# nomic-ai/contrastors

Measured on AMD Instinct MI355X. Metric: query-doc pairs/sec (whole node), nomic-bert-2048 seq128 global-batch 16384, higher is better.
Workload: dtype bf16

## Files before the change

contrastors_amd/csrc/gemm_bf16_v6.hip:

```cpp
#include "cx_common.h"
#include "../../include/contrastors_hip.h"
#include "gemm_params.h"
#include <type_traits>

namespace {

#ifndef CX_V6_HI_EARLY
#define CX_V6_HI_EARLY 1
#endif
#ifndef CX_V6_OPAQUE
#define CX_V6_OPAQUE 1
#endif
#ifndef CX_V6_NT
#define CX_V6_NT 3
#endif
template <int J>
__device__ __forceinline__ void v6_dma_m0(uint32_t slot_base) {
    asm volatile("s_add_u32 m0, %0, %1" ::"s"(slot_base), "n"(J * 4096) : "memory", "scc");
}
__device__ __forceinline__ void v6_dma_ld(uint32_t off, const bf16_t* base) {
    asm volatile("global_load_lds_dwordx4 %0, %1" ::"v"(off), "s"(base) : "memory");
}
template <int J>
__device__ __forceinline__ void v6_dma_full(uint32_t slot_base, uint32_t off, const bf16_t* base) {
    asm volatile("s_add_u32 m0, %0, %1\n\ts_nop 0\n\tglobal_load_lds_dwordx4 %2, %3" ::"s"(slot_base), "n"(J * 4096), "v"(off),
                 "s"(base) : "memory", "scc");
}
typedef unsigned int cx_u32x4 __attribute__((ext_vector_type(4)));
__device__ __forceinline__ void gst_nt(void* ptr, uint4 v) {
    cx_u32x4 t = {v.x, v.y, v.z, v.w};
    __builtin_nontemporal_store(t, reinterpret_cast<cx_u32x4*>(ptr));
}
__device__ __forceinline__ uint4 gld_nt(const void* ptr) {
    const cx_u32x4 t = __builtin_nontemporal_load(reinterpret_cast<const cx_u32x4*>(ptr));
    return make_uint4(t.x, t.y, t.z, t.w);
}
#if CX_V6_NT & 1
#define gst(ptr, v) gst_nt((ptr), (v))
#else
#define gst(ptr, v) (*reinterpret_cast<uint4*>(ptr) = (v))
#endif
#if CX_V6_NT & 2
#define gld(ptr) gld_nt(ptr)
#else
#define gld(ptr) (*reinterpret_cast<const uint4*>(ptr))
#endif

typedef __attribute__((address_space(3))) void* lds_void_ptr;
typedef const __attribute__((address_space(1))) void* glb_void_ptr;

constexpr int BM6 = 256, BN6 = 256, BK6 = 64;
constexpr int XS6 = 32768;
constexpr int LDS6 = 5 * XS6;

struct Frags6 {
    bf16x8_t w[8], x[8];
};

#include "gemm_v6_acc.inc"

template <int I0, int I1, class F>
CX_DEVICE void v6_static_for(F&& f) {
    if constexpr (I0 < I1) {
        f(std::integral_constant<int, I0>{});
        v6_static_for<I0 + 1, I1>(f);
    }
}

template <int EPI, int DBG = 0>
__global__ __launch_bounds__(256, 1) __attribute__((amdgpu_waves_per_eu(1, 1))) void gemm_bf16_v6_kernel(GemmParams p) {
    extern __shared__ __attribute__((aligned(16))) char dsm[];
    constexpr bool IS_SWIGLU_BWD = EPI == GEMM_EPI_SWIGLU_BWD || EPI == GEMM_EPI_SWIGLU_BWD_AG;
    constexpr bool AG = EPI == GEMM_EPI_SWIGLU_BWD_AG;
    constexpr bool SAVEG = EPI == GEMM_EPI_SWIGLU_G;
    long long t_begin = 0, n_ktiles = 0;
    if constexpr (DBG != 0) t_begin = (long long)__builtin_amdgcn_s_memtime();
    long long ph[9] = {0, 0, 0, 0, 0, 0, 0, 0, 0}, t_last = t_begin, kt0_cyc = 0;
#define CX_PH(i_)                                                              \
    do {                                                                       \
        if constexpr ((DBG & 128) != 0) {                                      \
            const long long now_ = (long long)__builtin_amdgcn_s_memtime();    \
            ph[(i_)] += now_ - t_last;                                         \
            t_last = now_;                                                     \
        }                                                                      \
    } while (0)
    const int tid = threadIdx.x;
    const int lane = tid & 63;
    const int wave = __builtin_amdgcn_readfirstlane(tid >> 6);
    const int l15 = lane & 15, g4 = lane >> 4;
    const int wm = wave >> 1, wn = wave & 1;
    const int nk = p.K / BK6;
    const int per_xcd = gridDim.x >> 3;
    const int xcd = blockIdx.x & 7, idx = blockIdx.x >> 3;
    const int gn = p.sup_n > 0 ? p.sup_n : 1, gm = 8 / gn;
    const int xi = xcd / gn, xj = xcd - xi * gn;
    const int m_lo = p.tiles_m * xi / gm, m_hi = p.tiles_m * (xi + 1) / gm;
    const int n_lo = p.tiles_n * xj / gn, n_wd = p.tiles_n * (xj + 1) / gn - n_lo;
    const int nloc = (m_hi - m_lo) * n_wd;
    auto tile_of = [&](int round) {
        const int l = round * per_xcd + idx;
        if (l >= nloc) return -1;
        const int q = l / n_wd;
        return ((m_lo + q) << 8) | (n_lo + (l - q * n_wd));
    };

    uint32_t xoff[8], woff[8];
    const bf16_t* xbase = p.X;
    const bf16_t* wbase = p.W;
    int lx_round = 0, lx_kt = 0, lx_slot = 0;
    int lw_round = 0, lw_kt = 0, lw_slot = 0;
    bool lx_live, lw_live;
    const int first_tile = tile_of(0);
    bool x_clamped = true, w_clamped = true;
    auto x_setup = [&](int tile) {
        const int tm = tile >> 8;
        xbase = p.X + (size_t)tm * BM6 * p.ldx;
        const int rows = p.M - tm * BM6;
        if (rows < BM6 || x_clamped) {
            x_clamped = rows < BM6;
#pragma unroll
            for (int j = 0; j < 8; ++j) {
                const int r = (j * 4 + wave) * 8 + (lane >> 3);
                const int c = (lane & 7) ^ ((r >> 1) & 7);
                const int rr = r < rows ? r : rows - 1;
                xoff[j] = (uint32_t)rr * (uint32_t)p.ldx * 2u + c * 16;
            }
        }
    };
    auto w_setup = [&](int tile) {
        const int tn = tile & 255;
        wbase = p.W + (size_t)tn * BN6 * p.ldw;
        const int rows = p.N - tn * BN6;
        if (rows < BN6 || w_clamped) {
            w_clamped = rows < BN6;
#pragma unroll
            for (int j = 0; j < 8; ++j) {
                const int r = (j * 4 + wave) * 8 + (lane >> 3);
                const int c = (lane & 7) ^ ((r >> 1) & 7);
                const int rr = r < rows ? r : rows - 1;
                woff[j] = (uint32_t)rr * (uint32_t)p.ldw * 2u + c * 16;
            }
        }
    };
    const uint32_t lds0 = (uint32_t)(uintptr_t)(lds_void_ptr)dsm;
    const uint32_t lds_wave = lds0 + wave * 1024;
    uint32_t x_m0 = lds_wave, w_m0 = lds_wave + 3 * XS6;
    auto issue_x_tile = [&]() {
        if constexpr ((DBG & 1) != 0) return;
        v6_dma_full<0>(x_m0, xoff[0], xbase); v6_dma_full<1>(x_m0, xoff[1], xbase); v6_dma_full<2>(x_m0, xoff[2], xbase);
        v6_dma_full<3>(x_m0, xoff[3], xbase); v6_dma_full<4>(x_m0, xoff[4], xbase); v6_dma_full<5>(x_m0, xoff[5], xbase);
        v6_dma_full<6>(x_m0, xoff[6], xbase); v6_dma_full<7>(x_m0, xoff[7], xbase);
    };
    auto issue_w_tile = [&]() {
        if constexpr ((DBG & 1) != 0) return;
        v6_dma_full<0>(w_m0, woff[0], wbase); v6_dma_full<1>(w_m0, woff[1], wbase); v6_dma_full<2>(w_m0, woff[2], wbase);
        v6_dma_full<3>(w_m0, woff[3], wbase); v6_dma_full<4>(w_m0, woff[4], wbase); v6_dma_full<5>(w_m0, woff[5], wbase);
        v6_dma_full<6>(w_m0, woff[6], wbase); v6_dma_full<7>(w_m0, woff[7], wbase);
    };
    auto x_advance = [&]() {
        xbase += BK6;
        lx_slot = lx_slot == 2 ? 0 : lx_slot + 1;
        x_m0 = lds_wave + lx_slot * XS6;
        if (++lx_kt == nk) {
            lx_kt = 0;
            const int t = tile_of(++lx_round);
            lx_live = t >= 0;
            x_setup(lx_live ? t : first_tile);
        }
    };
    auto w_advance = [&]() {
        wbase += BK6;
        lw_slot ^= 1;
        w_m0 = lds_wave + (3 + lw_slot) * XS6;
        if (++lw_kt == nk) {
            lw_kt = 0;
            const int t = tile_of(++lw_round);
            lw_live = t >= 0;
            w_setup(lw_live ? t : first_tile);
        }
    };


    int cp_round = 0;
    int cp_tile = first_tile;
    lx_live = lw_live = cp_tile >= 0;
    if (cp_tile < 0) return;
    x_setup(cp_tile);
    w_setup(cp_tile);
    issue_x_tile();
    x_advance();
    issue_w_tile();
    w_advance();
    issue_x_tile();
    x_advance();
    int xs_slot = 0, ws_slot = 0;

    Frags6 F0, F1;
    auto read_one = [&](Frags6& f, const char* xs, const char* ws, int kk, int i) {
        if constexpr ((DBG & 4) != 0) return;
        if (i < 8)
            f.w[i] = lds_read_frag(ws, tile64_off(wn * 128 + i * 16 + l15, kk * 4 + g4));
        else
            f.x[i - 8] = lds_read_frag(xs, tile64_off(wm * 128 + (i - 8) * 16 + l15, kk * 4 + g4));
    };
    auto mma1 = [&](const Frags6& f, int i) {
        if constexpr ((DBG & 8) != 0) return;
        v6_mfma(i, f.w[i & 7], f.x[i >> 3]);
    };
    auto mma1z = [&](const Frags6& f, int i) {
        if constexpr ((DBG & 8) != 0) return;
        v6_mfma_z(i, f.w[i & 7], f.x[i >> 3]);
    };

#ifndef CX_V6_DMA_SPREAD
#define CX_V6_DMA_SPREAD 4
#endif
#ifndef CX_V6_RD_SPREAD
#define CX_V6_RD_SPREAD 2
#endif
#define CX_SEG(MMA, f, i0, i1, nxt, rxs, rws, rkk, R0, RSP, kind, D0, DSP, J0, ND)                     \
    do {                                                                                              \
        v6_static_for<(i0), (i1)>([&](auto ic_) __attribute__((always_inline)) {                      \
            constexpr int I_ = decltype(ic_)::value;                                                  \
            constexpr bool RD_ = (RSP) > 0 && I_ >= (R0) && (I_ - (R0)) % ((RSP) > 0 ? (RSP) : 1) == 0 && (I_ - (R0)) / ((RSP) > 0 ? (RSP) : 1) < 16; \
            constexpr bool DM_ = (ND) > 0 && I_ >= (D0) && (I_ - (D0)) % (DSP) == 0 && (I_ - (D0)) / (DSP) < (ND); \
            constexpr int J_ = DM_ ? (J0) + (I_ - (D0)) / (DSP) : 0;                                  \
            if constexpr (RD_) read_one(nxt, rxs, rws, rkk, (I_ - (R0)) / ((RSP) > 0 ? (RSP) : 1));   \
            if constexpr (DM_) CX_DMA_M0(kind, J_);                                                   \
            MMA(f, I_);                                                                               \
            if constexpr (DM_) CX_DMA_LD(kind, J_);                                                   \
            __builtin_amdgcn_sched_barrier(0);                                                        \
        });                                                                                           \
    } while (0)
#define CX_DMA_M0(kind, J)                                                       \
    do {                                                                         \
        if constexpr ((kind) == 1 && (DBG & 1) == 0) v6_dma_m0<(J)>(w_m0);        \
        if constexpr ((kind) == 2 && (DBG & 1) == 0) v6_dma_m0<(J)>(x_m0);        \
    } while (0)
#define CX_DMA_LD(kind, J)                                                       \
    do {                                                                         \
        if constexpr ((kind) == 1 && (DBG & 1) == 0) v6_dma_ld(woff[(J)], wbase); \
        if constexpr ((kind) == 2 && (DBG & 1) == 0) v6_dma_ld(xoff[(J)], xbase); \
    } while (0)

    {
        asm volatile("s_waitcnt vmcnt(8)" ::: "memory");
        __builtin_amdgcn_s_barrier();
#pragma unroll
        for (int i = 0; i < 16; ++i) read_one(F0, dsm, dsm + 3 * XS6, 0, i);
    }

    int cp_kt = 0;
    int pxs_slot = 0, pws_slot = 0;
    auto kt_body = [&](auto first) {
        if constexpr (DBG != 0) ++n_ktiles;
        constexpr int RS_ = CX_V6_RD_SPREAD, DS_ = CX_V6_DMA_SPREAD;
        const char* xs = dsm + xs_slot * XS6;
        const char* ws = dsm + (3 + ws_slot) * XS6;
        const int nxs_slot = xs_slot == 2 ? 0 : xs_slot + 1, nws_slot = ws_slot ^ 1;
        if constexpr (decltype(first)::value) {
            CX_SEG(mma1z, F0, 0, 64, F1, xs, ws, 1, RS_ == 2 ? 0 : 1, RS_, 1, RS_ == 2 ? 1 : 17, DS_, 0, 8);
        } else {
            CX_SEG(mma1, F0, 0, 64, F1, xs, ws, 1, RS_ == 2 ? 0 : 1, RS_, 1, RS_ == 2 ? 1 : 17, DS_, 0, 8);
        }
        w_advance();
        CX_SEG(mma1, F1, 0, 32, F0, xs, ws, 0, 0, 0, 2, 0, RS_ == 2 ? 8 : DS_, 0, 4);
        asm volatile("s_waitcnt lgkmcnt(0)" ::: "memory");
        if constexpr ((DBG & 128) != 0) {
            const long long w0_ = (long long)__builtin_amdgcn_s_memtime();
            asm volatile("s_waitcnt vmcnt(4)" ::: "memory");
            const long long w1_ = (long long)__builtin_amdgcn_s_memtime();
            ph[decltype(first)::value ? 0 : 1] += w1_ - w0_;
        } else if constexpr ((DBG & 32) == 0) {
            asm volatile("s_waitcnt vmcnt(4)" ::: "memory");
        }
        if constexpr ((DBG & 2) == 0) __builtin_amdgcn_s_barrier();
        const char* nxs = dsm + nxs_slot * XS6;
        const char* nws = dsm + (3 + nws_slot) * XS6;
        CX_SEG(mma1, F1, 32, 64, F0, nxs, nws, 0, RS_ == 2 ? 32 : 33, RS_, 2, RS_ == 2 ? 33 : 49, RS_ == 2 ? 8 : DS_, 4, 4);
        x_advance();
        if constexpr ((DBG & 128) != 0 && decltype(first)::value) {
            const long long now_ = (long long)__builtin_amdgcn_s_memtime();
            kt0_cyc += now_ - t_last;
        }
        ++cp_kt;
        pxs_slot = xs_slot;
        pws_slot = ws_slot;
        xs_slot = nxs_slot;
        ws_slot = nws_slot;
    };

#pragma unroll 1
    while (cp_tile >= 0) {
        cp_kt = 0;
        kt_body(std::true_type{});
#pragma unroll 1
        while (cp_kt < nk) kt_body(std::false_type{});

        {
            CX_PH(2);
            asm volatile("s_nop 7\n\ts_nop 7\n\ts_nop 7" ::: "memory");
            const int tn = cp_tile & 255, tm = cp_tile >> 8;
            const int m0 = tm * BM6 + wm * 128, n0 = tn * BN6 + wn * 128;
            char* my = ((wave < 2) ? dsm + pxs_slot * XS6 : dsm + (3 + pws_slot) * XS6) + (wave & 1) * 16384;
            constexpr int ROWB = 272;
            auto prow = [&](int q) { return (q >> 1) * 16 + l15; };
            auto pcol = [&](int q) { return (q & 1) * 16 + 4 * g4; };
            auto qoff = [](int q, int rowb) { return (q >> 1) * 16 * rowb + (q & 1) * 32; };
            if constexpr ((DBG & 16) != 0) {
            } else if constexpr (EPI == GEMM_EPI_NONE || EPI == GEMM_EPI_ACT_BWD || EPI == GEMM_EPI_QACT_BWD) {
                constexpr bool ACTB = EPI == GEMM_EPI_ACT_BWD || EPI == GEMM_EPI_QACT_BWD;
                float cs0 = 0.f, cs1 = 0.f, cs2 = 0.f, cs3 = 0.f, cs4 = 0.f, cs5 = 0.f, cs6 = 0.f, cs7 = 0.f;
                constexpr int act_kind = EPI == GEMM_EPI_QACT_BWD ? CX_ACT_QUICK_GELU : CX_ACT_GELU;
                auto mul_grad = [&](uint4& v, const uint4& r) {
#define CX_MG(w_, ca, cb)                                                                              \
    {                                                                                                 \
        const float o0 = bf16lo_to_f32(v.w_) * act_grad(bf16lo_to_f32(r.w_), act_kind);               \
        const float o1 = bf16hi_to_f32(v.w_) * act_grad(bf16hi_to_f32(r.w_), act_kind);               \
        v.w_ = pack_bf16x2(o0, o1);                                                                   \
        ca += bf16lo_to_f32(v.w_);                                                                    \
        cb += bf16hi_to_f32(v.w_);                                                                    \
    }
                    CX_MG(x, cs0, cs1) CX_MG(y, cs2, cs3) CX_MG(z, cs4, cs5) CX_MG(w, cs6, cs7)
#undef CX_MG
                };
                auto flush_colsum = [&]() {
                    if constexpr (ACTB) {
                        float c[8] = {cs0, cs1, cs2, cs3, cs4, cs5, cs6, cs7};
#pragma unroll
                        for (int e = 0; e < 8; ++e) {
                            c[e] += __shfl_xor(c[e], 16, 64);
                            c[e] += __shfl_xor(c[e], 32, 64);
                        }
                        const int n = n0 + (lane & 15) * 8;
                        if (p.colsum_part && lane < 16 && m0 < p.M && n + 8 <= p.N) {
                            float* dst = p.colsum_part + (size_t)(m0 >> 7) * p.N + n;
                            *reinterpret_cast<float4*>(dst) = make_float4(c[0], c[1], c[2], c[3]);
                            *reinterpret_cast<float4*>(dst + 4) = make_float4(c[4], c[5], c[6], c[7]);
                        }
                    }
                };
                const bool add_bias = p.bias != nullptr;
                const bf16_t* resid = reinterpret_cast<const bf16_t*>(p.Out2);
                auto fast_tile = [&](auto with_resid) {
                    constexpr bool RES = decltype(with_resid)::value;
                    const int rrow = lane >> 4, rch = lane & 15;
                    bf16_t* outp = reinterpret_cast<bf16_t*>(p.Out) + (size_t)(m0 + rrow) * p.ldo + n0 + rch * 8;
                    const bf16_t* resp = RES ? resid + (size_t)(m0 + rrow) * p.ldo2 + n0 + rch * 8 : nullptr;
                    const char* rd = my + rrow * ROWB + rch * 16;
                    char* wr = my + prow(0) * ROWB + pcol(0) * 2;
                    uint2 pk[16];
                    auto pack_pass = [&](int b) {
#pragma unroll
                        for (int a = 0; a < 4; ++a) {
                            float blk[16];
                            v6_read_block(4 * b + a, blk);
#pragma unroll
                            for (int q = 0; q < 4; ++q) {
                                pk[a * 4 + q].x = pack_bf16x2(blk[4 * q], blk[4 * q + 1]);
                                pk[a * 4 + q].y = pack_bf16x2(blk[4 * q + 2], blk[4 * q + 3]);
                            }
                        }
                    };
                    auto stage = [&]() {
#pragma unroll
                        for (int a = 0; a < 4; ++a)
#pragma unroll
                            for (int q = 0; q < 4; ++q) *reinterpret_cast<uint2*>(wr + a * 64 + qoff(q, ROWB)) = pk[a * 4 + q];
                    };
                    uint4 r0 = {}, r1 = {}, r2 = {}, r3 = {}, r4 = {}, r5 = {}, r6 = {}, r7 = {};
#define CX_RES_ROWS(b_)                                                                                   \
    r0 = gld(resp + (size_t)((b_) * 32 + 0) * p.ldo2);                          \
    r1 = gld(resp + (size_t)((b_) * 32 + 4) * p.ldo2);                          \
    r2 = gld(resp + (size_t)((b_) * 32 + 8) * p.ldo2);                          \
    r3 = gld(resp + (size_t)((b_) * 32 + 12) * p.ldo2);                         \
    r4 = gld(resp + (size_t)((b_) * 32 + 16) * p.ldo2);                         \
    r5 = gld(resp + (size_t)((b_) * 32 + 20) * p.ldo2);                         \
    r6 = gld(resp + (size_t)((b_) * 32 + 24) * p.ldo2);                         \
    r7 = gld(resp + (size_t)((b_) * 32 + 28) * p.ldo2);
                    auto add_res = [&](uint4& v, const uint4& r) {
                        v.x = pack_bf16x2(bf16lo_to_f32(v.x) + bf16lo_to_f32(r.x), bf16hi_to_f32(v.x) + bf16hi_to_f32(r.x));
                        v.y = pack_bf16x2(bf16lo_to_f32(v.y) + bf16lo_to_f32(r.y), bf16hi_to_f32(v.y) + bf16hi_to_f32(r.y));
                        v.z = pack_bf16x2(bf16lo_to_f32(v.z) + bf16lo_to_f32(r.z), bf16hi_to_f32(v.z) + bf16hi_to_f32(r.z));
                        v.w = pack_bf16x2(bf16lo_to_f32(v.w) + bf16lo_to_f32(r.w), bf16hi_to_f32(v.w) + bf16hi_to_f32(r.w));
                    };
                    auto one_pass = [&](auto bc) {
                        constexpr int b = decltype(bc)::value;
                        uint4 v0 = *reinterpret_cast<const uint4*>(rd + 0 * ROWB), v1 = *reinterpret_cast<const uint4*>(rd + 4 * ROWB),
                              v2 = *reinterpret_cast<const uint4*>(rd + 8 * ROWB), v3 = *reinterpret_cast<const uint4*>(rd + 12 * ROWB),
                              v4 = *reinterpret_cast<const uint4*>(rd + 16 * ROWB), v5 = *reinterpret_cast<const uint4*>(rd + 20 * ROWB),
                              v6 = *reinterpret_cast<const uint4*>(rd + 24 * ROWB), v7 = *reinterpret_cast<const uint4*>(rd + 28 * ROWB);
                        __builtin_amdgcn_sched_barrier(0);
                        if constexpr (b < 3) pack_pass(b + 1);
                        __builtin_amdgcn_sched_barrier(0);
                        if constexpr (RES) {
                            add_res(v0, r0); add_res(v1, r1); add_res(v2, r2); add_res(v3, r3);
                            add_res(v4, r4); add_res(v5, r5); add_res(v6, r6); add_res(v7, r7);
                            if constexpr (b < 3) {
                                __builtin_amdgcn_sched_barrier(0);
                                CX_RES_ROWS(b + 1)
                                __builtin_amdgcn_sched_barrier(0);
                            }
                        }
                        if constexpr (b < 3) stage();
                        bf16_t* o = outp + (size_t)(b * 32) * p.ldo;
                        if constexpr ((DBG & 64) != 0) {
                            const uint4 vs[8] = {v0, v1, v2, v3, v4, v5, v6, v7};
#pragma unroll
                            for (int i = 0; i < 8; ++i) asm volatile("" ::"v"(vs[i].x), "v"(vs[i].y), "v"(vs[i].z), "v"(vs[i].w));
                            asm volatile("" ::"v"(o));
                            return;
                        }
                        gst(o, v0);
                        gst(o + (size_t)4 * p.ldo, v1);
                        gst(o + (size_t)8 * p.ldo, v2);
                        gst(o + (size_t)12 * p.ldo, v3);
                        gst(o + (size_t)16 * p.ldo, v4);
                        gst(o + (size_t)20 * p.ldo, v5);
                        gst(o + (size_t)24 * p.ldo, v6);
                        gst(o + (size_t)28 * p.ldo, v7);
                    };
                    if constexpr (RES) { CX_RES_ROWS(0) }
                    pack_pass(0);
                    stage();
                    one_pass(std::integral_constant<int, 0>{});
                    one_pass(std::integral_constant<int, 1>{});
                    one_pass(std::integral_constant<int, 2>{});
                    one_pass(std::integral_constant<int, 3>{});
#undef CX_RES_ROWS
                };
                auto fast_tile_actb = [&]() {
                    const int rrow = lane >> 4, rch = lane & 15;
                    bf16_t* outp = reinterpret_cast<bf16_t*>(p.Out) + (size_t)(m0 + rrow) * p.ldo + n0 + rch * 8;
                    const bf16_t* resp = resid + (size_t)(m0 + rrow) * p.ldo2 + n0 + rch * 8;
                    const char* rd = my + rrow * ROWB + rch * 16;
                    char* wr = my + prow(0) * ROWB + pcol(0) * 2;
                    auto stage_pass = [&](int b) {
#pragma unroll
                        for (int a = 0; a < 4; ++a) {
                            float blk[16];
                            v6_read_block(4 * b + a, blk);
#pragma unroll
                            for (int q = 0; q < 4; ++q) {
                                uint2 pk2;
                                pk2.x = pack_bf16x2(blk[4 * q], blk[4 * q + 1]);
                                pk2.y = pack_bf16x2(blk[4 * q + 2], blk[4 * q + 3]);
                                *reinterpret_cast<uint2*>(wr + a * 64 + qoff(q, ROWB)) = pk2;
                            }
                            __builtin_amdgcn_sched_barrier(0);
                        }
                    };
                    uint4 r0, r1, r2, r3;
#define CX_PRE_ROWS(hh_)                                                        \
    r0 = gld(resp + (size_t)((hh_) * 16 + 0) * p.ldo2);                         \
    r1 = gld(resp + (size_t)((hh_) * 16 + 4) * p.ldo2);                         \
    r2 = gld(resp + (size_t)((hh_) * 16 + 8) * p.ldo2);                         \
    r3 = gld(resp + (size_t)((hh_) * 16 + 12) * p.ldo2);
                    auto half_pass = [&](auto hc) {
                        constexpr int hh = decltype(hc)::value;
                        constexpr int h = hh & 1;
                        uint4 v0 = *reinterpret_cast<const uint4*>(rd + (h * 16 + 0) * ROWB), v1 = *reinterpret_cast<const uint4*>(rd + (h * 16 + 4) * ROWB),
                              v2 = *reinterpret_cast<const uint4*>(rd + (h * 16 + 8) * ROWB), v3 = *reinterpret_cast<const uint4*>(rd + (h * 16 + 12) * ROWB);
                        __builtin_amdgcn_sched_barrier(0);
                        mul_grad(v0, r0); __builtin_amdgcn_sched_barrier(0);
                        mul_grad(v1, r1); __builtin_amdgcn_sched_barrier(0);
                        mul_grad(v2, r2); __builtin_amdgcn_sched_barrier(0);
                        mul_grad(v3, r3); __builtin_amdgcn_sched_barrier(0);
                        if constexpr (hh < 7) { CX_PRE_ROWS(hh + 1) }
                        __builtin_amdgcn_sched_barrier(0);
                        bf16_t* o = outp + (size_t)(hh * 16) * p.ldo;
                        gst(o, v0);
                        gst(o + (size_t)4 * p.ldo, v1);
                        gst(o + (size_t)8 * p.ldo, v2);
                        gst(o + (size_t)12 * p.ldo, v3);
                        if constexpr (h == 1 && hh < 7) stage_pass((hh >> 1) + 1);
                    };
                    CX_PRE_ROWS(0)
                    stage_pass(0);
                    half_pass(std::integral_constant<int, 0>{}); half_pass(std::integral_constant<int, 1>{});
                    half_pass(std::integral_constant<int, 2>{}); half_pass(std::integral_constant<int, 3>{});
                    half_pass(std::integral_constant<int, 4>{}); half_pass(std::integral_constant<int, 5>{});
                    half_pass(std::integral_constant<int, 6>{}); half_pass(std::integral_constant<int, 7>{});
#undef CX_PRE_ROWS
                };
                const bool fast = p.alpha == 1.f && !add_bias && m0 + 128 <= p.M && n0 + 128 <= p.N;
                auto store_tile = [&](auto plain) {
#pragma unroll
                    for (int b = 0; b < 4; ++b) {
                        uint4 r0 = {}, r1 = {}, r2 = {}, r3 = {}, r4 = {}, r5 = {}, r6 = {}, r7 = {};
                        if (resid) {
#define CX_RES_LOAD(ps, dst)                                                                              \
    {                                                                                                 \
        int m_ = m0 + b * 32 + (ps) * 4 + (lane >> 4);                                                \
        m_ = m_ < p.M ? m_ : p.M - 1;                                                                 \
        int n_ = n0 + (lane & 15) * 8;                                                                \
        n_ = n_ + 8 <= p.N ? n_ : 0;                                                                  \
        dst = gld(resid + (size_t)m_ * p.ldo2 + n_);                      \
    }
                            CX_RES_LOAD(0, r0) CX_RES_LOAD(1, r1) CX_RES_LOAD(2, r2) CX_RES_LOAD(3, r3)
                            CX_RES_LOAD(4, r4) CX_RES_LOAD(5, r5) CX_RES_LOAD(6, r6) CX_RES_LOAD(7, r7)
#undef CX_RES_LOAD
                        }
#pragma unroll
                        for (int a = 0; a < 4; ++a) {
                            float blk[16];
                            v6_read_block(4 * b + a, blk);
#pragma unroll
                            for (int q = 0; q < 4; ++q) {
                                const int nl = a * 32 + pcol(q);
                                float v[4];
#pragma unroll
                                for (int e = 0; e < 4; ++e) v[e] = blk[4 * q + e];
                                if constexpr (!decltype(plain)::value) {
#pragma unroll
                                    for (int e = 0; e < 4; ++e) v[e] *= p.alpha;
                                    if (add_bias) {
                                        const int n = n0 + nl;
                                        if (n < p.N) {
                                            const float4 bv = *reinterpret_cast<const float4*>(p.bias + n);
                                            v[0] += bv.x; v[1] += bv.y; v[2] += bv.z; v[3] += bv.w;
                                        }
                                    }
                                }
                                uint2 pk;
                                pk.x = pack_bf16x2(v[0], v[1]);
                                pk.y = pack_bf16x2(v[2], v[3]);
                                *reinterpret_cast<uint2*>(my + prow(q) * ROWB + nl * 2) = pk;
                            }
                        }
#pragma unroll
                        for (int ps = 0; ps < 8; ++ps) {
                            const int row = ps * 4 + (lane >> 4), ch = lane & 15;
                            const int m = m0 + b * 32 + row, n = n0 + ch * 8;
                            uint4 vv = *reinterpret_cast<const uint4*>(my + row * ROWB + ch * 16);
                            if (resid && ACTB) {
                                const uint4 rr = ps == 0 ? r0 : ps == 1 ? r1 : ps == 2 ? r2 : ps == 3 ? r3 : ps == 4 ? r4 : ps == 5 ? r5
                                                 : ps == 6 ? r6 : r7;
                                if (m < p.M && n + 8 <= p.N) mul_grad(vv, rr);
                            } else if (resid) {
                                const uint4 rr = ps == 0 ? r0 : ps == 1 ? r1 : ps == 2 ? r2 : ps == 3 ? r3 : ps == 4 ? r4 : ps == 5 ? r5
                                                 : ps == 6 ? r6 : r7;
                                vv.x = pack_bf16x2(bf16lo_to_f32(vv.x) + bf16lo_to_f32(rr.x), bf16hi_to_f32(vv.x) + bf16hi_to_f32(rr.x));
                                vv.y = pack_bf16x2(bf16lo_to_f32(vv.y) + bf16lo_to_f32(rr.y), bf16hi_to_f32(vv.y) + bf16hi_to_f32(rr.y));
                                vv.z = pack_bf16x2(bf16lo_to_f32(vv.z) + bf16lo_to_f32(rr.z), bf16hi_to_f32(vv.z) + bf16hi_to_f32(rr.z));
                                vv.w = pack_bf16x2(bf16lo_to_f32(vv.w) + bf16lo_to_f32(rr.w), bf16hi_to_f32(vv.w) + bf16hi_to_f32(rr.w));
                            }
                            if (m < p.M && n + 8 <= p.N)
                                gst(reinterpret_cast<bf16_t*>(p.Out) + (size_t)m * p.ldo + n, vv);
                        }
                    }
                };
                if constexpr (ACTB) {
                    if (fast) {
                        fast_tile_actb();
                    } else {
                        store_tile(std::true_type{});
                    }
                    flush_colsum();
                } else if (fast) {
                    if (resid) {
                        fast_tile(std::true_type{});
                    } else {
                        fast_tile(std::false_type{});
                    }
                } else if (p.alpha == 1.f && !add_bias) {
                    store_tile(std::true_type{});
                } else {
                    store_tile(std::false_type{});
                }
            } else if constexpr (IS_SWIGLU_BWD) {
                const bf16_t* yg_in = reinterpret_cast<const bf16_t*>(p.Out2);
                const bf16_t* g_in = reinterpret_cast<const bf16_t*>(p.In3);
                bf16_t* dyg = reinterpret_cast<bf16_t*>(p.Out);
                const int c0 = 2 * n0;
                auto bwd_elem = [&](float yv, float gv, float dv, float& dyo, float& dgo) {
                    if constexpr (AG) {
                        swiglu_bwd_from_act(dv, yv, gv, dyo, dgo);
                    } else {
                        const float sg = __builtin_amdgcn_rcpf(1.f + __builtin_amdgcn_exp2f(-1.4426950408889634f * gv));
                        const float gs = gv * sg;
                        dyo = gs * dv;
                        dgo = (sg + gs * (1.f - sg)) * dv * yv;
                    }
                };
                auto bwd_quad = [&](const float (&yv)[4], const float (&gv)[4], const float* dv, float (&dyo)[4], float (&dgo)[4]) {
                    if constexpr (AG) {
#pragma unroll
                        for (int h = 0; h < 2; ++h) {
                            cx_f2 y2, g2;
                            swiglu_bwd_from_act2(cx_f2{dv[2 * h], dv[2 * h + 1]}, cx_f2{yv[2 * h], yv[2 * h + 1]},
                                                 cx_f2{gv[2 * h], gv[2 * h + 1]}, y2, g2);
                            dyo[2 * h] = y2.x; dyo[2 * h + 1] = y2.y;
                            dgo[2 * h] = g2.x; dgo[2 * h + 1] = g2.y;
                        }
                    } else {
#pragma unroll
                        for (int e = 0; e < 4; ++e) bwd_elem(yv[e], gv[e], dv[e], dyo[e], dgo[e]);
                    }
                };
                auto cell = [&](int row, int colbyte) { return my + row * 512 + ((((colbyte >> 4) ^ row) & 31) << 4) + (colbyte & 15); };
                const bool fast_bwd = m0 + 128 <= p.M && n0 + 128 <= p.N;
                if (fast_bwd) {
                    int lane_e = lane;
#if CX_V6_OPAQUE >= 1
                    asm volatile("" : "+v"(lane_e));
#endif
                    const int lrow = lane_e >> 5, lch = lane_e & 31;
                    const bf16_t* src = AG ? ((lch & 4) ? g_in : yg_in) + (size_t)(m0 + lrow) * p.ldo2 + n0 + (lch >> 3) * 32 + (lch & 3) * 8
                                           : yg_in + (size_t)(m0 + lrow) * p.ldo2 + c0 + lch * 8;
                    bf16_t* dst = dyg + (size_t)(m0 + lrow) * p.ldo + c0 + lch * 8;
                    uint4 t0, t1, t2, t3, t4, t5, t6, t7, t8, t9, t10, t11, t12, t13, t14, t15;
#define CX_L(i, b_) t##i = gld(src + (size_t)((b_) * 32 + (i) * 2) * p.ldo2);
#define CX_LOAD_LO(b_) CX_L(0, b_) CX_L(1, b_) CX_L(2, b_) CX_L(3, b_) CX_L(4, b_) CX_L(5, b_) CX_L(6, b_) CX_L(7, b_)
#define CX_LOAD_HI(b_) CX_L(8, b_) CX_L(9, b_) CX_L(10, b_) CX_L(11, b_) CX_L(12, b_) CX_L(13, b_) CX_L(14, b_) CX_L(15, b_)
#define CX_S(i) *reinterpret_cast<uint4*>(cell((i) * 2 + lrow, lch * 16)) = t##i;
#define CX_STAGE_ALL CX_S(0) CX_S(1) CX_S(2) CX_S(3) CX_S(4) CX_S(5) CX_S(6) CX_S(7) CX_S(8) CX_S(9) CX_S(10) CX_S(11) CX_S(12) CX_S(13) CX_S(14) CX_S(15)
                    auto one_pass = [&](auto bc) {
                        constexpr int b = decltype(bc)::value;
                        int lane_p = lane_e;
#if CX_V6_OPAQUE >= 2
                        asm volatile("" : "+v"(lane_p));
#endif
                        const int lrow = lane_p >> 5, lch = lane_p & 31, l15 = lane_p & 15, g4 = lane_p >> 4;
                        CX_STAGE_ALL
                        __builtin_amdgcn_sched_barrier(0);
                        CX_PH(4);
                        if constexpr (b < 3) { CX_LOAD_LO(b + 1) }
#if CX_V6_HI_EARLY
                        if constexpr (b < 3) { CX_LOAD_HI(b + 1) }
#endif
                        __builtin_amdgcn_sched_barrier(0);
                        CX_PH(5);
#pragma unroll
                        for (int a = 0; a < 4; ++a) {
                            float da[16];
                            v6_read_block(4 * b + a, da);
                            uint2 yy[4], gg[4];
#pragma unroll
                            for (int q = 0; q < 4; ++q) {
                                yy[q] = *reinterpret_cast<const uint2*>(cell((q >> 1) * 16 + l15, (a * 64 + (q & 1) * 16 + 4 * g4) * 2));
                                gg[q] = *reinterpret_cast<const uint2*>(cell((q >> 1) * 16 + l15, (a * 64 + 32 + (q & 1) * 16 + 4 * g4) * 2));
                            }
#pragma unroll
                            for (int q = 0; q < 4; ++q) {
                                char* py = cell((q >> 1) * 16 + l15, (a * 64 + (q & 1) * 16 + 4 * g4) * 2);
                                char* pg = cell((q >> 1) * 16 + l15, (a * 64 + 32 + (q & 1) * 16 + 4 * g4) * 2);
                                const float y[4] = {bf16lo_to_f32(yy[q].x), bf16hi_to_f32(yy[q].x), bf16lo_to_f32(yy[q].y), bf16hi_to_f32(yy[q].y)};
                                const float g[4] = {bf16lo_to_f32(gg[q].x), bf16hi_to_f32(gg[q].x), bf16lo_to_f32(gg[q].y), bf16hi_to_f32(gg[q].y)};
                                float dy[4], dg[4];
                                bwd_quad(y, g, &da[4 * q], dy, dg);
                                uint2 o;
                                o.x = pack_bf16x2(dy[0], dy[1]); o.y = pack_bf16x2(dy[2], dy[3]);
                                *reinterpret_cast<uint2*>(py) = o;
                                o.x = pack_bf16x2(dg[0], dg[1]); o.y = pack_bf16x2(dg[2], dg[3]);
                                *reinterpret_cast<uint2*>(pg) = o;
                            }
                            __builtin_amdgcn_sched_barrier(0);
                        }
#if !CX_V6_HI_EARLY
                        if constexpr (b < 3) { CX_LOAD_HI(b + 1) }
#endif
                        __builtin_amdgcn_sched_barrier(0);
                        CX_PH(6);
#pragma unroll
                        for (int h = 0; h < 4; ++h) {
                            const uint4 v0 = *reinterpret_cast<const uint4*>(cell((h * 4 + 0) * 2 + lrow, lch * 16));
                            const uint4 v1 = *reinterpret_cast<const uint4*>(cell((h * 4 + 1) * 2 + lrow, lch * 16));
                            const uint4 v2 = *reinterpret_cast<const uint4*>(cell((h * 4 + 2) * 2 + lrow, lch * 16));
                            const uint4 v3 = *reinterpret_cast<const uint4*>(cell((h * 4 + 3) * 2 + lrow, lch * 16));
                            bf16_t* o = dst + (size_t)(b * 32 + h * 8) * p.ldo;
                            gst(o, v0);
                            gst(o + (size_t)2 * p.ldo, v1);
                            gst(o + (size_t)4 * p.ldo, v2);
                            gst(o + (size_t)6 * p.ldo, v3);
                        }
                        __builtin_amdgcn_sched_barrier(0);
                        CX_PH(7);
                    };
                    CX_LOAD_LO(0) CX_LOAD_HI(0)
                    __builtin_amdgcn_sched_barrier(0);
                    CX_PH(3);
                    one_pass(std::integral_constant<int, 0>{});
                    one_pass(std::integral_constant<int, 1>{});
                    one_pass(std::integral_constant<int, 2>{});
                    one_pass(std::integral_constant<int, 3>{});
#undef CX_L
#undef CX_LOAD_LO
#undef CX_LOAD_HI
#undef CX_S
#undef CX_STAGE_ALL
                } else
#pragma unroll 1
                for (int b = 0; b < 4; ++b) {
                    int lane_c = lane;
                    asm volatile("" : "+v"(lane_c));
                    const int lrow = lane_c >> 5, lch = lane_c & 31, l15 = lane_c & 15, g4 = lane_c >> 4;
#define CX_YG_LOAD(i)                                                                                   \
    uint4 in##i;                                                                                      \
    {                                                                                                 \
        int m_ = m0 + b * 32 + (i) * 2 + lrow;                                                        \
        m_ = m_ < p.M ? m_ : p.M - 1;                                                                 \
        in##i = AG ? *reinterpret_cast<const uint4*>(((lch & 4) ? g_in : yg_in) + (size_t)m_ * p.ldo2 + n0 + (lch >> 3) * 32 + (lch & 3) * 8) \
                   : *reinterpret_cast<const uint4*>(yg_in + (size_t)m_ * p.ldo2 + c0 + lch * 8);     \
    }
#define CX_YG_STAGE(i) *reinterpret_cast<uint4*>(cell((i) * 2 + lrow, lch * 16)) = in##i;
                    {
                        CX_YG_LOAD(0) CX_YG_LOAD(1) CX_YG_LOAD(2) CX_YG_LOAD(3) CX_YG_LOAD(4) CX_YG_LOAD(5) CX_YG_LOAD(6)
                        CX_YG_LOAD(7)
                        CX_YG_STAGE(0) CX_YG_STAGE(1) CX_YG_STAGE(2) CX_YG_STAGE(3) CX_YG_STAGE(4) CX_YG_STAGE(5)
                        CX_YG_STAGE(6) CX_YG_STAGE(7)
                    }
                    {
                        CX_YG_LOAD(8) CX_YG_LOAD(9) CX_YG_LOAD(10) CX_YG_LOAD(11) CX_YG_LOAD(12) CX_YG_LOAD(13)
                        CX_YG_LOAD(14) CX_YG_LOAD(15)
                        CX_YG_STAGE(8) CX_YG_STAGE(9) CX_YG_STAGE(10) CX_YG_STAGE(11) CX_YG_STAGE(12) CX_YG_STAGE(13)
                        CX_YG_STAGE(14) CX_YG_STAGE(15)
                    }
#undef CX_YG_LOAD
#undef CX_YG_STAGE
#pragma unroll
                    for (int a = 0; a < 4; ++a) {
                        float da[16];
                        v6_read_block(4 * b + a, da);
#pragma unroll
                        for (int q = 0; q < 4; ++q) {
                            char* py = cell((q >> 1) * 16 + l15, (a * 64 + (q & 1) * 16 + 4 * g4) * 2);
                            char* pg = cell((q >> 1) * 16 + l15, (a * 64 + 32 + (q & 1) * 16 + 4 * g4) * 2);
                            const uint2 yy = *reinterpret_cast<const uint2*>(py);
                            const uint2 gg = *reinterpret_cast<const uint2*>(pg);
                            const float y[4] = {bf16lo_to_f32(yy.x), bf16hi_to_f32(yy.x), bf16lo_to_f32(yy.y), bf16hi_to_f32(yy.y)};
                            const float g[4] = {bf16lo_to_f32(gg.x), bf16hi_to_f32(gg.x), bf16lo_to_f32(gg.y), bf16hi_to_f32(gg.y)};
                            float dy[4], dg[4];
                            bwd_quad(y, g, &da[4 * q], dy, dg);
                            uint2 o;
                            o.x = pack_bf16x2(dy[0], dy[1]); o.y = pack_bf16x2(dy[2], dy[3]);
                            *reinterpret_cast<uint2*>(py) = o;
                            o.x = pack_bf16x2(dg[0], dg[1]); o.y = pack_bf16x2(dg[2], dg[3]);
                            *reinterpret_cast<uint2*>(pg) = o;
                        }
                    }
#pragma unroll
                    for (int i = 0; i < 16; ++i) {
                        const int row = i * 2 + lrow, ch = lch;
                        const int m = m0 + b * 32 + row;
                        const uint4 vv = *reinterpret_cast<const uint4*>(cell(row, ch * 16));
                        if (m < p.M) gst(dyg + (size_t)m * p.ldo + c0 + ch * 8, vv);
                    }
                }
            } else if constexpr (EPI == GEMM_EPI_GELU || EPI == GEMM_EPI_QGELU) {
                constexpr int act_kind = EPI == GEMM_EPI_QGELU ? CX_ACT_QUICK_GELU : CX_ACT_GELU;
                auto fast_gelu = [&](auto save_c) {
                    constexpr bool SAVE = decltype(save_c)::value;
                    const int rrow = lane >> 4, rch = lane & 15;
                    bf16_t* prep = SAVE ? reinterpret_cast<bf16_t*>(p.Out) + (size_t)(m0 + rrow) * p.ldo + n0 + rch * 8 : nullptr;
                    bf16_t* actp = reinterpret_cast<bf16_t*>(p.Out2) + (size_t)(m0 + rrow) * p.ldo2 + n0 + rch * 8;
                    const char* rd = my + rrow * ROWB + rch * 16;
                    char* wr = my + prow(0) * ROWB + pcol(0) * 2;
                    float4 bq[8];
#pragma unroll
                    for (int a = 0; a < 4; ++a)
#pragma unroll
                        for (int h = 0; h < 2; ++h)
                            bq[2 * a + h] = p.bias ? *reinterpret_cast<const float4*>(p.bias + n0 + a * 32 + pcol(h)) : make_float4(0.f, 0.f, 0.f, 0.f);
                    uint2 pkp[16], pka[16];
                    auto part_a = [&](int b) {
#pragma unroll
                        for (int a = 0; a < 4; ++a) {
                            float blk[16];
                            v6_read_block(4 * b + a, blk);
#pragma unroll
                            for (int q = 0; q < 4; ++q) {
                                const float4 bv = bq[2 * a + (q & 1)];
                                pkp[a * 4 + q].x = pack_bf16x2(blk[4 * q] + bv.x, blk[4 * q + 1] + bv.y);
                                pkp[a * 4 + q].y = pack_bf16x2(blk[4 * q + 2] + bv.z, blk[4 * q + 3] + bv.w);
                            }
                        }
                    };
                    auto part_b = [&]() {
#pragma unroll
                        for (int i = 0; i < 16; ++i) {
                            const float v0 = bf16lo_to_f32(pkp[i].x), v1 = bf16hi_to_f32(pkp[i].x), v2 = bf16lo_to_f32(pkp[i].y), v3 = bf16hi_to_f32(pkp[i].y);
                            pka[i].x = pack_bf16x2(act_val(v0, act_kind), act_val(v1, act_kind));
                            pka[i].y = pack_bf16x2(act_val(v2, act_kind), act_val(v3, act_kind));
                        }
                    };
                    auto stage = [&](const uint2 (&pk)[16]) {
#pragma unroll
                        for (int a = 0; a < 4; ++a)
#pragma unroll
                            for (int q = 0; q < 4; ++q) *reinterpret_cast<uint2*>(wr + a * 64 + qoff(q, ROWB)) = pk[a * 4 + q];
                    };
#define CX_ROWS8                                                                                                      \
    uint4 v0 = *reinterpret_cast<const uint4*>(rd + 0 * ROWB), v1 = *reinterpret_cast<const uint4*>(rd + 4 * ROWB),    \
          v2 = *reinterpret_cast<const uint4*>(rd + 8 * ROWB), v3 = *reinterpret_cast<const uint4*>(rd + 12 * ROWB),   \
          v4 = *reinterpret_cast<const uint4*>(rd + 16 * ROWB), v5 = *reinterpret_cast<const uint4*>(rd + 20 * ROWB),  \
          v6 = *reinterpret_cast<const uint4*>(rd + 24 * ROWB), v7 = *reinterpret_cast<const uint4*>(rd + 28 * ROWB);  \
    __builtin_amdgcn_sched_barrier(0);
#define CX_STORE8(o_, ld_)                                                                                            \
    gst(o_, v0); gst(o_ + (size_t)4 * (ld_), v1); gst(o_ + (size_t)8 * (ld_), v2); gst(o_ + (size_t)12 * (ld_), v3);   \
    gst(o_ + (size_t)16 * (ld_), v4); gst(o_ + (size_t)20 * (ld_), v5); gst(o_ + (size_t)24 * (ld_), v6); gst(o_ + (size_t)28 * (ld_), v7);
                    auto one_pass = [&](auto bc) {
                        constexpr int b = decltype(bc)::value;
                        if constexpr (SAVE) {
                            {
                                CX_ROWS8
                                part_b();
                                __builtin_amdgcn_sched_barrier(0);
                                stage(pka);
                                bf16_t* o = prep + (size_t)(b * 32) * p.ldo;
                                CX_STORE8(o, p.ldo)
                            }
                            __builtin_amdgcn_sched_barrier(0);
                            {
                                CX_ROWS8
                                if constexpr (b < 3) part_a(b + 1);
                                __builtin_amdgcn_sched_barrier(0);
                                if constexpr (b < 3) stage(pkp);
                                bf16_t* o = actp + (size_t)(b * 32) * p.ldo2;
                                CX_STORE8(o, p.ldo2)
                            }
                        } else {
                            CX_ROWS8
                            if constexpr (b < 3) { part_a(b + 1); part_b(); }
                            __builtin_amdgcn_sched_barrier(0);
                            if constexpr (b < 3) stage(pka);
                            bf16_t* o = actp + (size_t)(b * 32) * p.ldo2;
                            CX_STORE8(o, p.ldo2)
                        }
                        __builtin_amdgcn_sched_barrier(0);
                    };
                    part_a(0);
                    if constexpr (SAVE) {
                        stage(pkp);
                    } else {
                        part_b();
                        stage(pka);
                    }
                    one_pass(std::integral_constant<int, 0>{});
                    one_pass(std::integral_constant<int, 1>{});
                    one_pass(std::integral_constant<int, 2>{});
                    one_pass(std::integral_constant<int, 3>{});
#undef CX_ROWS8
#undef CX_STORE8
                };
                if (m0 + 128 <= p.M && n0 + 128 <= p.N) {
                    if (p.Out) {
                        fast_gelu(std::true_type{});
                    } else {
                        fast_gelu(std::false_type{});
                    }
                } else
#pragma unroll
                for (int b = 0; b < 4; ++b) {
                    float pre[4][16];
#pragma unroll
                    for (int a = 0; a < 4; ++a) {
                        v6_read_block(4 * b + a, pre[a]);
#pragma unroll
                        for (int q = 0; q < 4; ++q) {
                            const int n = n0 + a * 32 + pcol(q);
                            float4 bv = make_float4(0.f, 0.f, 0.f, 0.f);
                            if (p.bias && n < p.N) bv = *reinterpret_cast<const float4*>(p.bias + n);
                            pre[a][4 * q] = bf16_to_f32(f32_to_bf16(pre[a][4 * q] + bv.x));
                            pre[a][4 * q + 1] = bf16_to_f32(f32_to_bf16(pre[a][4 * q + 1] + bv.y));
                            pre[a][4 * q + 2] = bf16_to_f32(f32_to_bf16(pre[a][4 * q + 2] + bv.z));
                            pre[a][4 * q + 3] = bf16_to_f32(f32_to_bf16(pre[a][4 * q + 3] + bv.w));
                        }
                    }
#pragma unroll
                    for (int which = 0; which < 2; ++which) {
                        bf16_t* outp = reinterpret_cast<bf16_t*>(which == 0 ? p.Out : p.Out2);
                        const int ldo = which == 0 ? p.ldo : p.ldo2;
                        if (!outp) continue;
#pragma unroll
                        for (int a = 0; a < 4; ++a)
#pragma unroll
                            for (int q = 0; q < 4; ++q) {
                                float v[4];
#pragma unroll
                                for (int e = 0; e < 4; ++e) {
                                    v[e] = pre[a][4 * q + e];
                                    if (which == 1) v[e] = act_val(v[e], EPI == GEMM_EPI_QGELU ? CX_ACT_QUICK_GELU : CX_ACT_GELU);
                                }
                                uint2 pk;
                                pk.x = pack_bf16x2(v[0], v[1]);
                                pk.y = pack_bf16x2(v[2], v[3]);
                                *reinterpret_cast<uint2*>(my + prow(q) * ROWB + (a * 32 + pcol(q)) * 2) = pk;
                            }
#pragma unroll
                        for (int ps = 0; ps < 8; ++ps) {
                            const int row = ps * 4 + (lane >> 4), ch = lane & 15;
                            const int m = m0 + b * 32 + row, n = n0 + ch * 8;
                            const uint4 vv = *reinterpret_cast<const uint4*>(my + row * ROWB + ch * 16);
                            if (m < p.M && n + 8 <= p.N)
                                gst(outp + (size_t)m * ldo + n, vv);
                        }
                    }
                }
            } else {
                constexpr int AROWB = 144;
                char* mya = my + 32 * ROWB;
                auto fast_swiglu = [&](auto save_c) {
                    constexpr bool SAVE = decltype(save_c)::value;
                    constexpr bool SAVE_YG = SAVE && !SAVEG;
                    constexpr bool SAVE_G = SAVE && SAVEG;
                    const int rrow = lane >> 4, rch = lane & 15;
                    const int arow = lane >> 3, ach = lane & 7;
                    bf16_t* ygp = SAVE_YG ? reinterpret_cast<bf16_t*>(p.Out) + (size_t)(m0 + rrow) * p.ldo + n0 + rch * 8 : nullptr;
                    bf16_t* gp = SAVE_G ? reinterpret_cast<bf16_t*>(p.Out) + (size_t)(m0 + arow) * p.ldo + (n0 >> 1) + ach * 8 : nullptr;
                    bf16_t* actp = reinterpret_cast<bf16_t*>(p.Out2) + (size_t)(m0 + arow) * p.ldo2 + (n0 >> 1) + ach * 8;
                    const char* rdy = my + rrow * ROWB + rch * 16;
                    const char* rda = mya + arow * AROWB + ach * 16;
                    const char* rdg = my + arow * AROWB + ach * 16;
                    char* wry = my + prow(0) * ROWB + pcol(0) * 2;
                    char* wra = mya + prow(0) * AROWB + pcol(0) * 2;
                    char* wrg = my + prow(0) * AROWB + pcol(0) * 2;
                    uint2 pky[SAVE_YG ? 16 : 1], pkg[SAVE_G ? 8 : 1], pka[8];
                    auto compute_pass = [&](int b) {
#pragma unroll
                        for (int pr = 0; pr < 2; ++pr) {
                            float yb[16], gb[16];
                            v6_read_block(4 * b + 2 * pr, yb);
                            v6_read_block(4 * b + 2 * pr + 1, gb);
#pragma unroll
                            for (int q = 0; q < 4; ++q) {
                                uint2 py, pg;
                                py.x = pack_bf16x2(yb[4 * q], yb[4 * q + 1]);
                                py.y = pack_bf16x2(yb[4 * q + 2], yb[4 * q + 3]);
                                pg.x = pack_bf16x2(gb[4 * q], gb[4 * q + 1]);
                                pg.y = pack_bf16x2(gb[4 * q + 2], gb[4 * q + 3]);
                                if constexpr (SAVE_YG) {
                                    pky[(2 * pr) * 4 + q] = py;
                                    pky[(2 * pr + 1) * 4 + q] = pg;
                                }
                                if constexpr (SAVE_G) pkg[pr * 4 + q] = pg;
                                const float yy[4] = {bf16lo_to_f32(py.x), bf16hi_to_f32(py.x), bf16lo_to_f32(py.y), bf16hi_to_f32(py.y)};
                                const float gg[4] = {bf16lo_to_f32(pg.x), bf16hi_to_f32(pg.x), bf16lo_to_f32(pg.y), bf16hi_to_f32(pg.y)};
                                float o[4];
#pragma unroll
                                for (int e = 0; e < 4; ++e) o[e] = gg[e] * yy[e] * __builtin_amdgcn_rcpf(1.f + __expf(-gg[e]));
                                pka[pr * 4 + q].x = pack_bf16x2(o[0], o[1]);
                                pka[pr * 4 + q].y = pack_bf16x2(o[2], o[3]);
                            }
                        }
                    };
                    auto stage = [&]() {
                        if constexpr (SAVE_YG) {
#pragma unroll
                            for (int a = 0; a < 4; ++a)
#pragma unroll
                                for (int q = 0; q < 4; ++q) *reinterpret_cast<uint2*>(wry + a * 64 + qoff(q, ROWB)) = pky[a * 4 + q];
                        }
                        if constexpr (SAVE_G) {
#pragma unroll
                            for (int pr = 0; pr < 2; ++pr)
#pragma unroll
                                for (int q = 0; q < 4; ++q) *reinterpret_cast<uint2*>(wrg + pr * 64 + qoff(q, AROWB)) = pkg[pr * 4 + q];
                        }
#pragma unroll
                        for (int pr = 0; pr < 2; ++pr)
#pragma unroll
                            for (int q = 0; q < 4; ++q) *reinterpret_cast<uint2*>(wra + pr * 64 + qoff(q, AROWB)) = pka[pr * 4 + q];
                    };
                    auto one_pass = [&](auto bc) {
                        constexpr int b = decltype(bc)::value;
                        uint4 v0 = {}, v1 = {}, v2 = {}, v3 = {}, v4 = {}, v5 = {}, v6 = {}, v7 = {};
                        if constexpr (SAVE_YG) {
                            v0 = *reinterpret_cast<const uint4*>(rdy + 0 * ROWB); v1 = *reinterpret_cast<const uint4*>(rdy + 4 * ROWB);
                            v2 = *reinterpret_cast<const uint4*>(rdy + 8 * ROWB); v3 = *reinterpret_cast<const uint4*>(rdy + 12 * ROWB);
                            v4 = *reinterpret_cast<const uint4*>(rdy + 16 * ROWB); v5 = *reinterpret_cast<const uint4*>(rdy + 20 * ROWB);
                            v6 = *reinterpret_cast<const uint4*>(rdy + 24 * ROWB); v7 = *reinterpret_cast<const uint4*>(rdy + 28 * ROWB);
                        }
                        if constexpr (SAVE_G) {
                            v0 = *reinterpret_cast<const uint4*>(rdg + 0 * AROWB); v1 = *reinterpret_cast<const uint4*>(rdg + 8 * AROWB);
                            v2 = *reinterpret_cast<const uint4*>(rdg + 16 * AROWB); v3 = *reinterpret_cast<const uint4*>(rdg + 24 * AROWB);
                        }
                        const uint4 a0 = *reinterpret_cast<const uint4*>(rda + 0 * AROWB), a1 = *reinterpret_cast<const uint4*>(rda + 8 * AROWB),
                                    a2 = *reinterpret_cast<const uint4*>(rda + 16 * AROWB), a3 = *reinterpret_cast<const uint4*>(rda + 24 * AROWB);
                        __builtin_amdgcn_sched_barrier(0);
                        CX_PH(4);
                        if constexpr (b < 3) compute_pass(b + 1);
                        __builtin_amdgcn_sched_barrier(0);
                        CX_PH(5);
                        if constexpr (b < 3) stage();
                        __builtin_amdgcn_sched_barrier(0);
                        CX_PH(6);
                        if constexpr (SAVE_YG) {
                            bf16_t* o = ygp + (size_t)(b * 32) * p.ldo;
                            gst(o, v0);
                            gst(o + (size_t)4 * p.ldo, v1);
                            gst(o + (size_t)8 * p.ldo, v2);
                            gst(o + (size_t)12 * p.ldo, v3);
                            gst(o + (size_t)16 * p.ldo, v4);
                            gst(o + (size_t)20 * p.ldo, v5);
// ... 431 lines not shown
```

Before: 4352.

## Stream SwiGLU-backward y/g tiles into LDS via direct DMA ring

In the fused GEMM+SwiGLU-backward epilogue's fast path, the y/g operand tiles are now fetched with global_load_lds_dwordx4 straight into a 4-slot LDS ring, with swizzled source addressing. The previous path loaded them into VGPRs and then staged them into LDS. Units are processed in 16 steps with vmcnt-based waits, so the loads for later units overlap the compute and stores of earlier ones. Accumulators are read with explicit v_accvgpr_read instructions that hardcode AGPR indices. This removes a VGPR round-trip and register pressure, but it relies on exact accumulator register placement and hand-tuned waitcnt counts, which is fragile.

```diff
diff --git a/contrastors_amd/csrc/gemm_bf16_v6.hip b/contrastors_amd/csrc/gemm_bf16_v6.hip
--- a/contrastors_amd/csrc/gemm_bf16_v6.hip
+++ b/contrastors_amd/csrc/gemm_bf16_v6.hip
@@ -14,6 +14,9 @@
 #ifndef CX_V6_NT
 #define CX_V6_NT 3
 #endif
+#ifndef CX_V6_YG_DMA
+#define CX_V6_YG_DMA 1
+#endif
 template <int J>
 __device__ __forceinline__ void v6_dma_m0(uint32_t slot_base) {
     asm volatile("s_add_u32 m0, %0, %1" ::"s"(slot_base), "n"(J * 4096) : "memory", "scc");
@@ -25,6 +28,23 @@
 __device__ __forceinline__ void v6_dma_full(uint32_t slot_base, uint32_t off, const bf16_t* base) {
     asm volatile("s_add_u32 m0, %0, %1\n\ts_nop 0\n\tglobal_load_lds_dwordx4 %2, %3" ::"s"(slot_base), "n"(J * 4096), "v"(off),
                  "s"(base) : "memory", "scc");
+}
+template <int J, int OFF>
+__device__ __forceinline__ void v6_dma_row(uint32_t dst, const void* src) {
+#if CX_V6_NT & 2
+    asm volatile("s_add_u32 m0, %0, %1\n\ts_nop 0\n\tglobal_load_lds_dwordx4 %2, off offset:%3 nt" ::"s"(dst), "n"(J * 1024), "v"(src),
+                 "n"(OFF) : "memory", "scc");
+#else
+    asm volatile("s_add_u32 m0, %0, %1\n\ts_nop 0\n\tglobal_load_lds_dwordx4 %2, off offset:%3" ::"s"(dst), "n"(J * 1024), "v"(src),
+                 "n"(OFF) : "memory", "scc");
+#endif
+}
+template <int R0>
+__device__ __forceinline__ void v6_read_acc8(float (&t)[8]) {
+    asm volatile("v_accvgpr_read_b32 %0, a[%8]\n\tv_accvgpr_read_b32 %1, a[%9]\n\tv_accvgpr_read_b32 %2, a[%10]\n\tv_accvgpr_read_b32 %3, a[%11]\n\t"
+                 "v_accvgpr_read_b32 %4, a[%12]\n\tv_accvgpr_read_b32 %5, a[%13]\n\tv_accvgpr_read_b32 %6, a[%14]\n\tv_accvgpr_read_b32 %7, a[%15]"
+                 : "=v"(t[0]), "=v"(t[1]), "=v"(t[2]), "=v"(t[3]), "=v"(t[4]), "=v"(t[5]), "=v"(t[6]), "=v"(t[7])
+                 : "n"(R0), "n"(R0 + 1), "n"(R0 + 2), "n"(R0 + 3), "n"(R0 + 4), "n"(R0 + 5), "n"(R0 + 6), "n"(R0 + 7));
 }
 typedef unsigned int cx_u32x4 __attribute__((ext_vector_type(4)));
 __device__ __forceinline__ void gst_nt(void* ptr, uint4 v) {
@@ -600,6 +620,94 @@
                 };
                 auto cell = [&](int row, int colbyte) { return my + row * 512 + ((((colbyte >> 4) ^ row) & 31) << 4) + (colbyte & 15); };
                 const bool fast_bwd = m0 + 128 <= p.M && n0 + 128 <= p.N;
+#if CX_V6_YG_DMA
+                if (fast_bwd) {
+                    int lane_e = lane;
+                    asm volatile("" : "+v"(lane_e));
+                    const int drow = lane_e >> 4, dpc = lane_e & 15, l15 = lane_e & 15, g4 = lane_e >> 4;
+                    const uint32_t ring = (uint32_t)(uintptr_t)(lds_void_ptr)my;
+                    const bf16_t* ysrc[4];
+#pragma unroll
+                    for (int j = 0; j < 4; ++j) {
+                        const int lc = dpc ^ (4 * j + drow);
+                        ysrc[j] = AG ? ((lc & 4) ? g_in : yg_in) + (size_t)(m0 + 4 * j + drow) * p.ldo2 + n0 + (lc >> 3) * 32 + (lc & 3) * 8
+                                     : yg_in + (size_t)(m0 + 4 * j + drow) * p.ldo2 + c0 + lc * 8;
+                    }
+                    bf16_t* dst = dyg + (size_t)(m0 + drow) * p.ldo + c0 + dpc * 8;
+                    auto issue_unit = [&](auto uc) {
+                        constexpr int u = decltype(uc)::value, pp = u & 1;
+                        constexpr int PE = pp * (AG ? 64 : 128);
+                        const uint32_t slot = ring + (u & 3) * 4096;
+                        v6_dma_row<0, 0>(slot, ysrc[0] + PE);
+                        v6_dma_row<1, 0>(slot, ysrc[1] + PE);
+                        v6_dma_row<2, 0>(slot, ysrc[2] + PE);
+                        v6_dma_row<3, 0>(slot, ysrc[3] + PE);
+                        if constexpr (pp == 1) {
+#pragma unroll
+                            for (int j = 0; j < 4; ++j) ysrc[j] += (size_t)16 * p.ldo2;
+                        }
+                    };
+                    auto ucell = [&](char* s, int row, int colbyte) { return s + row * 256 + ((((colbyte >> 4) ^ row) & 15) << 4) + (colbyte & 15); };
+                    auto one_unit = [&](auto uc) {
+                        constexpr int u = decltype(uc)::value, b = u >> 2, h = (u >> 1) & 1, pp = u & 1;
+                        constexpr int YOUNGER = u < 4 ? 12 + 4 * u : 12 + 4 * (15 - u < 3 ? 15 - u : 3);
+                        char* s = my + (u & 3) * 4096;
+                        asm volatile("s_waitcnt vmcnt(%0)" ::"n"(YOUNGER) : "memory");
+                        __builtin_amdgcn_sched_barrier(0);
+                        CX_PH(4);
+                        v6_static_for<0, 2>([&](auto ac) __attribute__((always_inline)) {
+                            constexpr int a2 = decltype(ac)::value;
+                            float da[8];
+                            v6_read_acc8<16 * (4 * b + 2 * pp + a2) + 8 * h>(da);
+                            uint2 yy[2], gg[2];
+#pragma unroll
+                            for (int qq = 0; qq < 2; ++qq) {
+                                yy[qq] = *reinterpret_cast<const uint2*>(ucell(s, l15, a2 * 128 + qq * 32 + 8 * g4));
+                                gg[qq] = *reinterpret_cast<const uint2*>(ucell(s, l15, a2 * 128 + 64 + qq * 32 + 8 * g4));
+                            }
+#pragma unroll
+                            for (int qq = 0; qq < 2; ++qq) {
+                                const float y[4] = {bf16lo_to_f32(yy[qq].x), bf16hi_to_f32(yy[qq].x), bf16lo_to_f32(yy[qq].y), bf16hi_to_f32(yy[qq].y)};
+                                const float g[4] = {bf16lo_to_f32(gg[qq].x), bf16hi_to_f32(gg[qq].x), bf16lo_to_f32(gg[qq].y), bf16hi_to_f32(gg[qq].y)};
+                                float dy[4], dg[4];
+                                bwd_quad(y, g, &da[4 * qq], dy, dg);
+                                uint2 o;
+                                o.x = pack_bf16x2(dy[0], dy[1]); o.y = pack_bf16x2(dy[2], dy[3]);
+                                *reinterpret_cast<uint2*>(ucell(s, l15, a2 * 128 + qq * 32 + 8 * g4)) = o;
+                                o.x = pack_bf16x2(dg[0], dg[1]); o.y = pack_bf16x2(dg[2], dg[3]);
+                                *reinterpret_cast<uint2*>(ucell(s, l15, a2 * 128 + 64 + qq * 32 + 8 * g4)) = o;
+                            }
+                            __builtin_amdgcn_sched_barrier(0);
+                        });
+                        CX_PH(6);
+                        const uint4 v0 = *reinterpret_cast<const uint4*>(ucell(s, drow, dpc * 16));
+                        const uint4 v1 = *reinterpret_cast<const uint4*>(ucell(s, 4 + drow, dpc * 16));
+                        const uint4 v2 = *reinterpret_cast<const uint4*>(ucell(s, 8 + drow, dpc * 16));
+                        const uint4 v3 = *reinterpret_cast<const uint4*>(ucell(s, 12 + drow, dpc * 16));
+                        bf16_t* o = dst + pp * 128;
+                        gst(o, v0);
+                        gst(o + (size_t)4 * p.ldo, v1);
+                        gst(o + (size_t)8 * p.ldo, v2);
+                        gst(o + (size_t)12 * p.ldo, v3);
+                        if constexpr (pp == 1) dst += (size_t)16 * p.ldo;
+                        __builtin_amdgcn_sched_barrier(0);
+                        CX_PH(7);
+                        if constexpr (u + 4 < 16) {
+                            asm volatile("s_waitcnt lgkmcnt(0)" ::: "memory");
+                            issue_unit(std::integral_constant<int, u + 4>{});
+                        }
+                        __builtin_amdgcn_sched_barrier(0);
+                        CX_PH(5);
+                    };
+                    issue_unit(std::integral_constant<int, 0>{});
+                    issue_unit(std::integral_constant<int, 1>{});
+                    issue_unit(std::integral_constant<int, 2>{});
+                    issue_unit(std::integral_constant<int, 3>{});
+                    __builtin_amdgcn_sched_barrier(0);
+                    CX_PH(3);
+                    v6_static_for<0, 16>([&](auto uc) __attribute__((always_inline)) { one_unit(uc); });
+                } else
+#else
                 if (fast_bwd) {
                     int lane_e = lane;
 #if CX_V6_OPAQUE >= 1
@@ -690,6 +798,7 @@
 #undef CX_S
 #undef CX_STAGE_ALL
                 } else
+#endif
 #pragma unroll 1
                 for (int b = 0; b < 4; ++b) {
                     int lane_c = lane;
```

Result: no change. 4362 (median of 6 runs) (+0.2%).
